# Asd-g/AviSynth-JincResize

Hardware: AMD Instinct MI355X
Metric: Mpix/s per GPU (1080p→4K tap=3 Y8); % HBM-read roofline (higher is better)
Workload: dtype f32

## Files before the change

avisynth-jincresize_amd/csrc/kernel_periodic.hip:

```cpp
#include "device_common.hpp"
#include "knobs.h"
#include <utility>

#pragma clang fp contract(off)

namespace jinc {
namespace {

#include "kernel_periodic_common.inc"

constexpr int kTileCols = 64;

template <int FS, int RG = (FS <= 7 ? 8 : 9)>
struct PeriodicCfg {
    static constexpr int kRowGroups = RG;
    static constexpr int kTileRows = FS * kRowGroups;
    static constexpr int kLdsCols = kTileCols + FS;
    static constexpr int kLdsPitch = kLdsCols + 1;
    static constexpr int kLdsRows = kTileRows + FS;
};

template <typename T, int FS, int RG>
__global__ __launch_bounds__(256) void ewa_periodic_kernel(const PeriodicArgs a, const PlaneIO io) {
    using Cfg = PeriodicCfg<FS, RG>;
// ... 950 lines not shown
            : "v"(w1), "v"(w2), "v"(w3), "s"(c2), "s"(c3), "s"(c4), "s"(c5));
    }
}
#undef JINC_Q7_EVEN
#undef JINC_Q7_ODD

template <int SLOT>
__device__ __forceinline__ void quad2_load_row(f32x2 (&w)[24], const float* p) {
    const f32x2* p2 = reinterpret_cast<const f32x2*>(p);
#pragma unroll
    for (int m = 0; m < 4; ++m) w[4 * SLOT + m] = p2[m];
}

template <int U, uint32_t INNER, int NT>
__device__ __forceinline__ void quad2_pixel6(f32x2 (&acc)[4], const f32x2 (&w)[24], const JINC_CONSTANT f32x2* quad) {
    f32x2 ca[16], cb[16];
    quad_fetch(ca, quad, 0);
#define JINC_QUAD2_STEP(LY, CUR, NEXT)                                                                                        \
    if constexpr (LY < 5) quad_fetch(NEXT, quad, LY + 1);                                                                      \
    __builtin_amdgcn_sched_barrier(0);                                                                                         \
    quad_arrived(CUR);                                                                                                         \
    {                                                                                                                          \
        constexpr int S = 4 * ((U + LY) % 6);                                                                                  \
         \
        if constexpr (NT == 7) {                                             \
                                          \
            quad2_row7_span<(INNER >> (2 * (2 * LY))) & 3u>(acc[0], acc[1], w[S], w[S + 1], w[S + 2], w[S + 3], CUR[0], CUR[1], CUR[2], CUR[3], CUR[4], CUR[5], CUR[6]); \
            quad2_row7_span<(INNER >> (2 * (2 * LY + 1))) & 3u>(acc[2], acc[3], w[S], w[S + 1], w[S + 2], w[S + 3], CUR[8], CUR[9], CUR[10], CUR[11], CUR[12], CUR[13], CUR[14]); \
        } else {                                                                                                               \
        if constexpr ((INNER >> (2 * LY)) & 1u)                                                                                \
            quad2_row6_inner(acc[0], acc[1], w[S], w[S + 1], w[S + 2], CUR[1], CUR[2], CUR[3], CUR[4]);                        \
        else                                                                                                                   \
            quad2_row6(acc[0], acc[1], w[S], w[S + 1], w[S + 2], w[S + 3], CUR[0], CUR[1], CUR[2], CUR[3], CUR[4], CUR[5]);    \
        if constexpr ((INNER >> (2 * LY + 1)) & 1u)                                                                            \
            quad2_row6_inner(acc[2], acc[3], w[S], w[S + 1], w[S + 2], CUR[9], CUR[10], CUR[11], CUR[12]);                     \
        else                                                                                                                   \
            quad2_row6(acc[2], acc[3], w[S], w[S + 1], w[S + 2], w[S + 3], CUR[8], CUR[9], CUR[10], CUR[11], CUR[12], CUR[13]); \
        }                                                                                                                      \
    }                                                                                                                          \
    __builtin_amdgcn_sched_barrier(0);
    JINC_QUAD2_STEP(0, ca, cb)
    JINC_QUAD2_STEP(1, cb, ca)
    JINC_QUAD2_STEP(2, ca, cb)
    JINC_QUAD2_STEP(3, cb, ca)
    JINC_QUAD2_STEP(4, ca, cb)
    JINC_QUAD2_STEP(5, cb, ca)
#undef JINC_QUAD2_STEP
}

template <typename T>
__device__ __forceinline__ void store_quad_buf(BufferRsrc rsrc, uint32_t voffset, uint32_t soffset, f32x2 a, f32x2 b, float peak, bool b_ok) {
    if constexpr (std::is_same_v<T, float>) {
        typedef uint32_t u32x2 __attribute__((ext_vector_type(2)));
        __builtin_amdgcn_raw_buffer_store_b64(__builtin_bit_cast(u32x2, a), rsrc, voffset, soffset, 0);
        if (b_ok) __builtin_amdgcn_raw_buffer_store_b64(__builtin_bit_cast(u32x2, b), rsrc, voffset + 8u, soffset, 0);
    } else if constexpr (std::is_same_v<T, uint8_t>) {
        uint32_t w = __builtin_amdgcn_cvt_pk_u8_f32(a.x, 0u, 0u);
        w = __builtin_amdgcn_cvt_pk_u8_f32(a.y, 1u, w);
        w = __builtin_amdgcn_cvt_pk_u8_f32(b.x, 2u, w);
        w = __builtin_amdgcn_cvt_pk_u8_f32(b.y, 3u, w);
        if (b_ok) __builtin_amdgcn_raw_buffer_store_b32(w, rsrc, voffset, soffset, 0);
        else __builtin_amdgcn_raw_buffer_store_b16(static_cast<uint16_t>(w), rsrc, voffset, soffset, 0);
    } else {
        typedef uint32_t u32x2 __attribute__((ext_vector_type(2)));
        const uint32_t lo = round_pair16<T>(a.x, a.y, peak);
        if (b_ok) {
            const u32x2 v = {lo, round_pair16<T>(b.x, b.y, peak)};
            __builtin_amdgcn_raw_buffer_store_b64(v, rsrc, voffset, soffset, 0);
        } else {
            __builtin_amdgcn_raw_buffer_store_b32(lo, rsrc, voffset, soffset, 0);
        }
    }
}

template <typename T>
__device__ __forceinline__ bool edge_tile_of(const PeriodicArgs& a, int tile_x) {
    if constexpr (is_float_sample_v<T>) return false;
    return a.edge.coeffs != nullptr && ((a.edge.n[0] > 0 && tile_x == a.edge.tile_x[0]) || (a.edge.n[1] > 0 && tile_x == a.edge.tile_x[1]));
}

template <typename T, typename Cfg>
__device__ __forceinline__ void stage_edge_column(const PeriodicArgs& a, const PlaneIO& io, float* tile, int tile_x, const char* sbase, int gx0, int gy0,
                                                  int wave, int lane) {
    static_assert(Cfg::kLdsPitch >= Cfg::kLdsCols + 1 && Cfg::kLdsRows <= 64, "a spare word per tile row, one tile row per lane");
    const bool in_front = (a.edge.n[0] > 0 && tile_x == a.edge.tile_x[0] && a.edge.lds_col[0] < 0) || (a.edge.n[1] > 0 && tile_x == a.edge.tile_x[1] && a.edge.lds_col[1] < 0);
    if (in_front && wave == 0 && lane < Cfg::kLdsRows && gx0 > 0) {
        int gy = gy0 + lane;
        gy = gy < a.src_h ? gy : a.src_h - 1;
        tile[lane * Cfg::kLdsPitch - 1] = to_float(reinterpret_cast<const T*>(sbase + static_cast<size_t>(gy) * io.src_pitch)[gx0 - 1]);
    }
}

template <typename T, typename Cfg, int NR, int NC, int ES = 1>
__device__ __forceinline__ void quad2_edge_columns(const PeriodicArgs& a, const PlaneIO& io, const float* tile, int tile_x, int j0, int wave, int lane,
                                                   BufferRsrc drsrc) {
    constexpr int NCP = (NC + 3) & ~3;
    for (int s = 0; s < 2; ++s) {
        const int n = a.edge.n[s];
        if (n <= 0 || tile_x != a.edge.tile_x[s]) continue;
        const int q = wave & 1, half = (n + 1) >> 1;
        const int k_begin = (wave >> 1) * half, k_end = k_begin + half < n ? k_begin + half : n;
        if (k_begin >= k_end) continue;
        const bool live = lane < Cfg::kTileRows && j0 + lane < a.nj;
        static_assert(Cfg::kLdsRows <= 64, "one tile row per lane");
        const float* wp = tile + ((lane < Cfg::kLdsRows ? lane : 0) * Cfg::kLdsPitch + a.edge.lds_col[s]) * ES;
        float w[NR][NC];
#pragma unroll
        for (int lx = 0; lx < NC; ++lx) w[0][lx] = wp[lx * ES];
#pragma unroll
        for (int ly = 1; ly < NR; ++ly)
#pragma unroll
            for (int lx = 0; lx < NC; ++lx)
                w[ly][lx] = __builtin_bit_cast(float, __builtin_amdgcn_update_dpp(0, __builtin_bit_cast(int, w[ly - 1][lx]), 0x130, 0xf, 0xf, false));
        const uint32_t row_off = static_cast<uint32_t>(a.iy0 + 2 * (j0 + lane) + q) * static_cast<uint32_t>(io.dst_pitch);
        for (int k0 = k_begin; k0 < k_end; k0 += 4) {
            const int nk = k_end - k0 < 4 ? k_end - k0 : 4;
            float r[4];
#pragma unroll
            for (int k = 0; k < 4; ++k) {
                r[k] = 0.f;
                if (k < nk) {
                    const JINC_CONSTANT float* cs = (const JINC_CONSTANT float*)(a.edge.coeffs) + ((s * PeriodicArgs::EdgeColumns::kMaxPerSide + k0 + k) * 2 + q) * (NR * NCP);
                    float acc = 0.f;
#pragma unroll
                    for (int ly = 0; ly < NR; ++ly)
#pragma unroll
                        for (int lx = 0; lx < NC; ++lx) acc = acc + w[ly][lx] * cs[ly * NCP + lx];
                    r[k] = acc;
                }
            }
            if (!live) continue;
            const uint32_t voff = row_off + static_cast<uint32_t>(a.edge.x0[s] + k0) * static_cast<uint32_t>(sizeof(T));
            if (nk == 4) {
                if constexpr (std::is_same_v<T, uint8_t>) {
                    uint32_t v = __builtin_amdgcn_cvt_pk_u8_f32(r[0], 0u, 0u);
                    v = __builtin_amdgcn_cvt_pk_u8_f32(r[1], 1u, v);
                    v = __builtin_amdgcn_cvt_pk_u8_f32(r[2], 2u, v);
                    v = __builtin_amdgcn_cvt_pk_u8_f32(r[3], 3u, v);
                    __builtin_amdgcn_raw_buffer_store_b32(v, drsrc, voff, 0, 0);
                } else {
                    typedef uint32_t u32x2 __attribute__((ext_vector_type(2)));
                    const u32x2 v = {round_pair_u16(r[0], r[1], io.peak), round_pair_u16(r[2], r[3], io.peak)};
                    __builtin_amdgcn_raw_buffer_store_b64(v, drsrc, voff, 0, 0);
                }
            } else {
#pragma unroll
                for (int k = 0; k < 3; ++k)
                    if (k < nk) store_sample_buf<T>(drsrc, voff + static_cast<uint32_t>(k * sizeof(T)), 0, r[k], io.peak);
            }
        }
    }
}

struct Quad2ShareCfg {
    static constexpr int kTileCols = 128;
    static constexpr int kBlocksPerWave = 2;
    static constexpr int kTileRows = 4 * 2 * kBlocksPerWave;
    static constexpr int kLdsCols = kTileCols + 6;
    static constexpr int kLdsPitch = 136;
    static constexpr int kLdsRows = kTileRows + 5;
    static constexpr int kLdsFloats = 2 * (2 + kLdsRows * kLdsPitch);
};

template <int RG>
__host__ __device__ inline bool quad2_share_runs(const PlaneIO& io) { return RG == 8 || io.nframes > 1; }

constexpr uint32_t quad2_share_outs(int r, int c, int k) {
    uint32_t m = 0;
    for (int oy = 0; oy < 4; ++oy)
        for (int ox = 0; ox < 4; ++ox) {
            const int ly = r - (oy >> 1), lx = c - (ox >> 1);
            if (ly < 0 || ly > 5 || lx < 0 || lx > 5) continue;
            if (quad2_share_class(quad2_share_m(ox & 1, lx), quad2_share_m(oy & 1, ly)) == k) m |= 1u << (4 * oy + ox);
        }
    return m;
}

template <int R, int C, int K>
__device__ __forceinline__ void quad2_share_mul(f32x2& t, f32x2 s, const f32x2 (&w)[kQuad2ShareClasses / 2]) {
    if constexpr (quad2_share_outs(R, C, K) != 0) {
        if constexpr (K & 1)
            asm("v_pk_mul_f32 %0, %1, %2 op_sel:[0,1] op_sel_hi:[1,1]" : "=v"(t) : "v"(s), "s"(w[K >> 1]));
        else
            asm("v_pk_mul_f32 %0, %1, %2 op_sel_hi:[1,0]" : "=v"(t) : "v"(s), "s"(w[K >> 1]));
    }
}
template <int R, int C, int K>
__device__ __forceinline__ void quad2_share_adds(f32x2 (&acc)[16], f32x2 t) {
    constexpr uint32_t outs = quad2_share_outs(R, C, K);
#pragma unroll
    for (int o = 0; o < 16; ++o)
        if constexpr (outs != 0)
            if ((outs >> o) & 1u) asm("v_pk_add_f32 %0, %0, %1" : "+v"(acc[o]) : "v"(t));
}
template <int R, int C, int... K>
__device__ __forceinline__ void quad2_share_sample(f32x2 (&acc)[16], f32x2 s, const f32x2 (&w)[kQuad2ShareClasses / 2], std::integer_sequence<int, K...>) {
    f32x2 t[kQuad2ShareClasses];
    (quad2_share_mul<R, C, K>(t[K], s, w), ...);
    (quad2_share_adds<R, C, K>(acc, t[K]), ...);
}
template <int R, int... C>
__device__ __forceinline__ void quad2_share_row(f32x2 (&acc)[16], const f32x2 (&row)[8], const f32x2 (&w)[kQuad2ShareClasses / 2], std::integer_sequence<int, C...>) {
    (quad2_share_sample<R, C>(acc, row[C], w, std::make_integer_sequence<int, kQuad2ShareClasses>{}), ...);
}

template <typename T>
__device__ __forceinline__ void quad2_share_body(const PeriodicArgs& a, const PlaneIO& io, float* lds) {
    using Cfg = Quad2ShareCfg;
    typedef float f32x4 __attribute__((ext_vector_type(4)));
    f32x2* const tile = reinterpret_cast<f32x2*>(lds) + 2;
    const int lane = threadIdx.x & 63;
    const int wave = __builtin_amdgcn_readfirstlane(threadIdx.x >> 6);
    int tile_x, tile_y;
    swizzled_tile(tile_x, tile_y);
    const int i0 = tile_x * Cfg::kTileCols;
    const int j0 = tile_y * Cfg::kTileRows;
    const size_t f0 = 2 * static_cast<size_t>(blockIdx.z);
    const bool f1_ok = f0 + 1 < static_cast<size_t>(io.nframes);
    const size_t f1 = f1_ok ? f0 + 1 : f0;
    const bool edge_tile = edge_tile_of<T>(a, tile_x);
    {
        const int gx0 = a.min_sx + i0;
        const int gy0 = a.min_sy + j0;
        const char* sb0 = static_cast<const char*>(io.src) + f0 * io.src_frame_stride;
        const char* sb1 = static_cast<const char*>(io.src) + f1 * io.src_frame_stride;
        constexpr int kRowsPerWave = (Cfg::kLdsRows + 3) / 4;
        constexpr int kColsPerLane = (Cfg::kLdsCols + 63) / 64;
        T s0[kRowsPerWave][kColsPerLane], s1[kRowsPerWave][kColsPerLane];
#pragma unroll
        for (int i = 0; i < kRowsPerWave; ++i) {
            int gy = gy0 + wave + 4 * i;
            gy = gy < a.src_h ? gy : a.src_h - 1;
            const T* r0 = reinterpret_cast<const T*>(sb0 + static_cast<size_t>(gy) * io.src_pitch);
            const T* r1 = reinterpret_cast<const T*>(sb1 + static_cast<size_t>(gy) * io.src_pitch);
#pragma unroll
            for (int k = 0; k < kColsPerLane; ++k) {
                int gx = gx0 + lane + 64 * k;
                gx = gx < a.src_w ? gx : a.src_w - 1;
                s0[i][k] = r0[gx];
                s1[i][k] = r1[gx];
            }
        }
#pragma unroll
        for (int i = 0; i < kRowsPerWave; ++i) {
            const int r = wave + 4 * i;
#pragma unroll
            for (int k = 0; k < kColsPerLane; ++k) {
                const int c = lane + 64 * k;
                if (r < Cfg::kLdsRows && c < Cfg::kLdsCols) tile[r * Cfg::kLdsPitch + c] = f32x2{to_float(s0[i][k]), to_float(s1[i][k])};
            }
        }
        const bool in_front = edge_tile && ((a.edge.n[0] > 0 && tile_x == a.edge.tile_x[0] && a.edge.lds_col[0] < 0) ||
                                            (a.edge.n[1] > 0 && tile_x == a.edge.tile_x[1] && a.edge.lds_col[1] < 0));
        if (in_front && wave == 0 && lane < Cfg::kLdsRows && gx0 > 0) {
            int gy = gy0 + lane;
            gy = gy < a.src_h ? gy : a.src_h - 1;
            tile[lane * Cfg::kLdsPitch - 1] = f32x2{to_float(reinterpret_cast<const T*>(sb0 + static_cast<size_t>(gy) * io.src_pitch)[gx0 - 1]),
                                                    to_float(reinterpret_cast<const T*>(sb1 + static_cast<size_t>(gy) * io.src_pitch)[gx0 - 1])};
        }
    }
    __syncthreads();
    const uint32_t plane_bytes = static_cast<uint32_t>(io.dst_pitch) * a.dst_h;
    const BufferRsrc d0 = make_rsrc(static_cast<char*>(io.dst) + f0 * io.dst_frame_stride, plane_bytes);
    const BufferRsrc d1 = make_rsrc(static_cast<char*>(io.dst) + f1 * io.dst_frame_stride, plane_bytes);
    if (edge_tile) {
        quad2_edge_columns<T, Cfg, 6, 7, 2>(a, io, reinterpret_cast<const float*>(tile), tile_x, j0, wave, lane, d0);
        if (f1_ok) quad2_edge_columns<T, Cfg, 6, 7, 2>(a, io, reinterpret_cast<const float*>(tile) + 1, tile_x, j0, wave, lane, d1);
    }
    const int ia = i0 + 2 * lane;
    if (ia >= a.ni) return;
    const bool b_ok = ia + 1 < a.ni;
    f32x2 w[kQuad2ShareClasses / 2];
#pragma unroll
    for (int k = 0; k < kQuad2ShareClasses / 2; ++k) w[k] = f32x2{a.share_w[2 * k], a.share_w[2 * k + 1]};
    const uint32_t xoff = static_cast<uint32_t>(a.ix0 + 2 * ia) * static_cast<uint32_t>(sizeof(T));
    for (int blk = 0; blk < Cfg::kBlocksPerWave; ++blk) {
        const int jb = 2 * (wave * Cfg::kBlocksPerWave + blk);
        if (j0 + jb >= a.nj) break;
        const f32x2* wb = tile + jb * Cfg::kLdsPitch + 2 * lane;
        f32x2 acc[16];
#pragma unroll
        for (int o = 0; o < 16; ++o) acc[o] = f32x2{0.f, 0.f};
#define JINC_SHARE_ROW(R)                                                                                 \
    {                                                                                                     \
        const f32x4* p4 = reinterpret_cast<const f32x4*>(wb + (R) * Cfg::kLdsPitch);                      \
        f32x2 row[8];                                                                                     \
        _Pragma("unroll") for (int m = 0; m < 4; ++m) {                                                   \
            const f32x4 v = p4[m];                                                                        \
            row[2 * m] = f32x2{v.x, v.y};                                                                 \
            row[2 * m + 1] = f32x2{v.z, v.w};                                                             \
        }                                                                                                 \
        quad2_share_row<R>(acc, row, w, std::make_integer_sequence<int, 7>{});                            \
    }
        JINC_SHARE_ROW(0) JINC_SHARE_ROW(1) JINC_SHARE_ROW(2) JINC_SHARE_ROW(3) JINC_SHARE_ROW(4) JINC_SHARE_ROW(5) JINC_SHARE_ROW(6)
#undef JINC_SHARE_ROW
#pragma unroll
        for (int pr = 0; pr < 2; ++pr) {
            const int j = j0 + jb + pr;
            if (j >= a.nj) break;
#pragma unroll
            for (int q = 0; q < 2; ++q) {
                const uint32_t so = static_cast<uint32_t>(a.iy0 + 2 * j + q) * static_cast<uint32_t>(io.dst_pitch);
                const f32x2* r = acc + 4 * (2 * pr + q);
                store_quad_buf<T>(d0, xoff, so, f32x2{r[0].x, r[1].x}, f32x2{r[2].x, r[3].x}, io.peak, b_ok);
                if (f1_ok) store_quad_buf<T>(d1, xoff, so, f32x2{r[0].y, r[1].y}, f32x2{r[2].y, r[3].y}, io.peak, b_ok);
            }
        }
    }
}

constexpr uint32_t kQuad2InnerTap3 = PeriodicArgs::kQuadInnerTap3;
template <typename T, int RG, uint32_t INNER, int NT = 6>
__global__ __launch_bounds__(256, 6) void ewa_periodic_quad2_kernel(const PeriodicArgs a, const PlaneIO io) {
    using Cfg = Quad2Cfg<RG>;
    constexpr int FS = Cfg::FS;
    static_assert(RG % 4 == 0, "the four waves of a workgroup take RG / 4 row groups each");
    constexpr bool kShare = !is_float_sample_v<T> && INNER == kQuad2InnerTap3 && NT == 6;
    constexpr int kWords = 2 + Cfg::kLdsRows * Cfg::kLdsPitch;
    if constexpr (kShare && RG == 8) {
        __shared__ __attribute__((aligned(16))) float share_words[Quad2ShareCfg::kLdsFloats];
        quad2_share_body<T>(a, io, share_words);
        return;
    }
    __shared__ __attribute__((aligned(16))) float tile_words[kShare && Quad2ShareCfg::kLdsFloats > kWords ? Quad2ShareCfg::kLdsFloats : kWords];
    if constexpr (kShare) {
        if (quad2_share_runs<RG>(io)) {
            quad2_share_body<T>(a, io, tile_words);
            return;
        }
    }
    float* const tile = tile_words + 2;

    const int lane = threadIdx.x & 63;
    const int wave = __builtin_amdgcn_readfirstlane(threadIdx.x >> 6);
    int tile_x, tile_y;
    swizzled_tile(tile_x, tile_y);
    const int i0 = tile_x * Cfg::kTileCols;
    const int j0 = tile_y * Cfg::kTileRows;
    const size_t frame = blockIdx.z;
    if (skips_frame(a, frame)) return;
    const bool edge_tile = edge_tile_of<T>(a, tile_x);
    {
        const int gx0 = a.min_sx + i0;
        const int gy0 = a.min_sy + j0;
        const char* sbase = static_cast<const char*>(io.src) + frame * io.src_frame_stride;
        constexpr int kRowsPerWave = (Cfg::kLdsRows + 3) / 4;
        constexpr int kColsPerLane = (Cfg::kLdsCols + 63) / 64;
        T staged[kRowsPerWave][kColsPerLane];
        NonFinite<T> nonfinite(a, frame);
#pragma unroll
        for (int i = 0; i < kRowsPerWave; ++i) {
            int gy = gy0 + wave + 4 * i;
            gy = gy < a.src_h ? gy : a.src_h - 1;
            const T* srow = reinterpret_cast<const T*>(sbase + static_cast<size_t>(gy) * io.src_pitch);
#pragma unroll
            for (int k = 0; k < kColsPerLane; ++k) {
                int gx = gx0 + lane + 64 * k;
                gx = gx < a.src_w ? gx : a.src_w - 1;
                staged[i][k] = srow[gx];
            }
        }
#pragma unroll
        for (int i = 0; i < kRowsPerWave; ++i) {
            const int r = wave + 4 * i;
#pragma unroll
            for (int k = 0; k < kColsPerLane; ++k) {
                const int c = lane + 64 * k;
                if (r < Cfg::kLdsRows && c < Cfg::kLdsCols) tile[r * Cfg::kLdsPitch + c] = nonfinite.take(staged[i][k]);
            }
        }
        if constexpr (!is_float_sample_v<T>) {
            if (edge_tile) stage_edge_column<T, Cfg>(a, io, tile, tile_x, sbase, gx0, gy0, wave, lane);
        }
    }
    __syncthreads();
    const BufferRsrc drsrc = make_rsrc(static_cast<char*>(io.dst) + frame * io.dst_frame_stride,
                                       static_cast<uint32_t>(io.dst_pitch) * a.dst_h);
    if constexpr (!is_float_sample_v<T>) {
        if (edge_tile) quad2_edge_columns<T, Cfg, 6, 7>(a, io, tile, tile_x, j0, wave, lane, drsrc);
    }
    const int ia = i0 + 2 * lane;
    if (ia >= a.ni) return;
    const bool b_ok = ia + 1 < a.ni;

    const JINC_CONSTANT f32x2* quad = (const JINC_CONSTANT f32x2*)(a.quad);
    const float* base = tile + 2 * lane;
    const uint32_t xoff = static_cast<uint32_t>(a.ix0 + 2 * ia) * static_cast<uint32_t>(sizeof(T));

    constexpr int kGroupsPerWave = RG / 4;
    const int g_first = wave * kGroupsPerWave;
    if (j0 + g_first * FS >= a.nj) return;
    f32x2 win[24];
    {
        const float* wb = base + (g_first * FS) * Cfg::kLdsPitch;
        quad2_load_row<0>(win, wb + 0 * Cfg::kLdsPitch);
        quad2_load_row<1>(win, wb + 1 * Cfg::kLdsPitch);
        quad2_load_row<2>(win, wb + 2 * Cfg::kLdsPitch);
        quad2_load_row<3>(win, wb + 3 * Cfg::kLdsPitch);
        quad2_load_row<4>(win, wb + 4 * Cfg::kLdsPitch);
    }
    for (int g = g_first; g < g_first + kGroupsPerWave; ++g) {
        if (j0 + g * FS >= a.nj) break;
        const float* gbase = base + (g * FS) * Cfg::kLdsPitch;
#define JINC_QUAD2_ROW(U)                                                                                          \
    {                                                                                                              \
        quad2_load_row<(U + FS - 1) % FS>(win, gbase + (U + FS - 1) * Cfg::kLdsPitch);                              \
        f32x2 acc[4] = {{0.f, 0.f}, {0.f, 0.f}, {0.f, 0.f}, {0.f, 0.f}};                                            \
        uint32_t zero;                                                                                              \
        asm volatile("s_mov_b32 %0, 0" : "=s"(zero));  \
        quad2_pixel6<U, INNER, NT>(acc, win, quad + zero);                                                          \
        const int j = j0 + g * FS + U;                                                                              \
        if (j < a.nj) {                                                                                             \
            const uint32_t so = static_cast<uint32_t>(a.iy0 + 2 * j) * io.dst_pitch;                                \
            store_quad_buf<T>(drsrc, xoff, so, acc[0], acc[1], io.peak, b_ok);                                      \
            store_quad_buf<T>(drsrc, xoff, so + static_cast<uint32_t>(io.dst_pitch), acc[2], acc[3], io.peak, b_ok); \
        }                                                                                                           \
    }
        JINC_QUAD2_ROW(0) JINC_QUAD2_ROW(1) JINC_QUAD2_ROW(2) JINC_QUAD2_ROW(3) JINC_QUAD2_ROW(4) JINC_QUAD2_ROW(5)
#undef JINC_QUAD2_ROW
    }
}

template <int RG>
struct Quad2x8Cfg {
    static constexpr int FS = 8;
    static constexpr int kTileCols = 128;
    static constexpr int kTileRows = FS * RG;
    static constexpr int kLdsCols = kTileCols + FS;
    static constexpr int kLdsPitch = 138;
    static constexpr int kLdsRows = kTileRows + FS - 1;
};

__device__ __forceinline__ void quad2_row8(f32x2& acc_a, f32x2& acc_b, f32x2 w0, f32x2 w1, f32x2 w2, f32x2 w3, f32x2 w4, f32x2 c0, f32x2 c1,
                                           f32x2 c2, f32x2 c3, f32x2 c4, f32x2 c5, f32x2 c6, f32x2 c7) {
    f32x2 ta, tb;
#define JINC_LO(T, W, C) "v_pk_mul_f32 " T ", " W ", " C " op_sel_hi:[0,1]\n\t"
#define JINC_HI(T, W, C) "v_pk_mul_f32 " T ", " W ", " C " op_sel:[1,0] op_sel_hi:[1,1]\n\t"
#define JINC_ADD2 "v_pk_add_f32 %0, %0, %2\n\tv_pk_add_f32 %1, %1, %3\n\t"
    asm(JINC_LO("%2", "%4", "%9") JINC_HI("%3", "%4", "%9") JINC_ADD2
        JINC_HI("%2", "%4", "%10") JINC_LO("%3", "%5", "%10") JINC_ADD2
        JINC_LO("%2", "%5", "%11") JINC_HI("%3", "%5", "%11") JINC_ADD2
        JINC_HI("%2", "%5", "%12") JINC_LO("%3", "%6", "%12") JINC_ADD2
        JINC_LO("%2", "%6", "%13") JINC_HI("%3", "%6", "%13") JINC_ADD2
        JINC_HI("%2", "%6", "%14") JINC_LO("%3", "%7", "%14") JINC_ADD2
        JINC_LO("%2", "%7", "%15") JINC_HI("%3", "%7", "%15") JINC_ADD2
        JINC_HI("%2", "%7", "%16") JINC_LO("%3", "%8", "%16")
        "v_pk_add_f32 %0, %0, %2\n\tv_pk_add_f32 %1, %1, %3"
        : "+v"(acc_a), "+v"(acc_b), "=&v"(ta), "=&v"(tb)
        : "v"(w0), "v"(w1), "v"(w2), "v"(w3), "v"(w4), "s"(c0), "s"(c1), "s"(c2), "s"(c3), "s"(c4), "s"(c5), "s"(c6), "s"(c7));
#undef JINC_LO
#undef JINC_HI
#undef JINC_ADD2
}

template <int SLOT>
__device__ __forceinline__ void quad2x8_load_row(f32x2 (&w)[40], const float* p) {
    const f32x2* p2 = reinterpret_cast<const f32x2*>(p);
#pragma unroll
    for (int m = 0; m < 5; ++m) w[5 * SLOT + m] = p2[m];
}

template <int U, uint32_t TR8>
__device__ __forceinline__ void quad2_pixel8(f32x2 (&acc)[4], const f32x2 (&w)[40], const JINC_CONSTANT f32x2* quad) {
    f32x2 ca[16], cb[16];
    quad_fetch(ca, quad, 0);
#define JINC_QUAD2X8_STEP(LY, CUR, NEXT)                                                                                                  \
    if constexpr (LY < 7) quad_fetch(NEXT, quad, LY + 1);                                                                                  \
    __builtin_amdgcn_sched_barrier(0);                                                                                                     \
    quad_arrived(CUR);                                                                                                                     \
    {                                                                                                                                      \
        constexpr int S = 5 * ((U + LY) % 8);                                                                                              \
        if constexpr (quad8_trim_of(TR8, LY, 0) == 2)                                                                                      \
            quad2_row8_t2(acc[0], acc[1], w[S + 1], w[S + 2], w[S + 3], CUR[2], CUR[3], CUR[4], CUR[5]);                                   \
        else if constexpr (quad8_trim_of(TR8, LY, 0) == 1)                                                                                 \
            quad2_row8_t1(acc[0], acc[1], w[S], w[S + 1], w[S + 2], w[S + 3], CUR[1], CUR[2], CUR[3], CUR[4], CUR[5], CUR[6]);             \
        else                                                                                                                               \
            quad2_row8(acc[0], acc[1], w[S], w[S + 1], w[S + 2], w[S + 3], w[S + 4], CUR[0], CUR[1], CUR[2], CUR[3], CUR[4], CUR[5],       \
                       CUR[6], CUR[7]);                                                                                                    \
        if constexpr (quad8_trim_of(TR8, LY, 1) == 2)                                                                                      \
            quad2_row8_t2(acc[2], acc[3], w[S + 1], w[S + 2], w[S + 3], CUR[10], CUR[11], CUR[12], CUR[13]);                               \
// ... 302 lines not shown
    if (skips_frame(a, frame)) return;

    {
        const int gx0 = a.min_sx + i0;
        const int gy0 = a.min_sy + j0;
        const char* sbase = static_cast<const char*>(io.src) + frame * io.src_frame_stride;
        constexpr int kRowsPerWave = (Cfg::kRows + Cfg::kWaves - 1) / Cfg::kWaves;
        constexpr int kColsPerLane = (Cfg::kCols + 63) / 64;
        T staged[kRowsPerWave][kColsPerLane];
        NonFinite<T> nonfinite(a, frame);
#pragma unroll
        for (int i = 0; i < kRowsPerWave; ++i) {
            int gy = gy0 + wave + Cfg::kWaves * i;
            gy = gy < a.src_h ? gy : a.src_h - 1;
            const T* srow = reinterpret_cast<const T*>(sbase + static_cast<size_t>(gy) * io.src_pitch);
#pragma unroll
            for (int k = 0; k < kColsPerLane; ++k) {
                int gx = gx0 + lane + 64 * k;
                gx = gx < a.src_w ? gx : a.src_w - 1;
                staged[i][k] = srow[gx];
            }
        }
#pragma unroll
        for (int i = 0; i < kRowsPerWave; ++i) {
            const int r = wave + Cfg::kWaves * i;
#pragma unroll
            for (int k = 0; k < kColsPerLane; ++k) {
                const int c = lane + 64 * k;
                if (r < Cfg::kRows && c < Cfg::kCols)
                    tile[(c % K) * Cfg::kPlaneStride + r * Cfg::kPlane + c / K] = nonfinite.take(staged[i][k]);
            }
        }
    }
    __syncthreads();

    const BufferRsrc dframe = make_rsrc(static_cast<char*>(io.dst) + frame * io.dst_frame_stride,
                                        static_cast<uint32_t>(io.dst_pitch) * a.dst_h);
    const int nphase = a.px * a.py;
    const int nitems = nphase * Cfg::kChunks;
    const int cols_valid = a.ni - (i0 + K * lane);
    if (cols_valid <= 0) return;
    for (int item = wave; item < nitems; item += Cfg::kWaves) {
        const int ch = item / nphase;
        const int ph = item - ch * nphase;
        const int q = ph / a.px;
        const int p = ph - q * a.px;
        const int j = j0 + ch * R;
        const int rows_valid = a.nj - j;
        if (rows_valid <= 0) continue;
        const int nrows = a.rows_ny ? a.rows_ny : FS;
        const JINC_CONSTANT float* cs =
            (const JINC_CONSTANT float*)(a.coeffs + static_cast<size_t>(a.set[ph]) * (static_cast<size_t>(nrows) * padded_row(FS)));
        const unsigned base = ((a.start_y[q] - a.min_sy) + ch * R) * Cfg::kPlane + lane;
        const int y0 = a.iy0 + a.py * j + q;
        const unsigned x0 = a.ix0 + a.px * (i0 + K * lane) + p;
        const JINC_CONSTANT int32_t* row_trim = a.row_trim ? (const JINC_CONSTANT int32_t*)(a.row_trim) + ph * 32 : nullptr;
        if (a.start_x[p] - a.min_sx)
            rows_item<T, FS, KC, 1>(tile, base, cs, row_trim, nrows, dframe, io.dst_pitch, io.peak, y0, a.py, rows_valid, x0, a.px, cols_valid);
        else
            rows_item<T, FS, KC, 0>(tile, base, cs, row_trim, nrows, dframe, io.dst_pitch, io.peak, y0, a.py, rows_valid, x0, a.px, cols_valid);
    }
}

template <typename T, int FS, int RG = PeriodicCfg<FS>::kRowGroups>
int launch_periodic_t(const PeriodicArgs& pa, const PlaneIO& io, hipStream_t stream) {
    using Cfg = PeriodicCfg<FS, RG>;
    dim3 grid((pa.ni + kTileCols - 1) / kTileCols, (pa.nj + Cfg::kTileRows - 1) / Cfg::kTileRows, io.nframes);
    hipLaunchKernelGGL((ewa_periodic_kernel<T, FS, RG>), grid, dim3(256, 1, 1), 0, stream, pa, io);
    knobs::note_instance("ewa_periodic_kernel", "%s, %d, %d", knobs::type_name<T>(), FS, RG);
    return static_cast<int>(hipGetLastError());
}

template <typename T, int FS, int RG>
int launch_periodic_pk_t(const PeriodicArgs& pa, const PlaneIO& io, hipStream_t stream) {
    using Cfg = PeriodicPkCfg<FS, RG>;
    dim3 grid((pa.ni + Cfg::kTileCols - 1) / Cfg::kTileCols, (pa.nj + Cfg::kTileRows - 1) / Cfg::kTileRows, io.nframes);
    hipLaunchKernelGGL((ewa_periodic_pk_kernel<T, FS, RG>), grid, dim3(256, 1, 1), 0, stream, pa, io);
    knobs::note_instance("ewa_periodic_pk_kernel", "%s, %d, %d", knobs::type_name<T>(), FS, RG);
    return static_cast<int>(hipGetLastError());
}

template <typename T, int RG>
int launch_periodic_quad_t(const PeriodicArgs& pa, const PlaneIO& io, hipStream_t stream) {
    using Cfg = PeriodicCfg<7, RG>;
    dim3 grid((pa.ni + kTileCols - 1) / kTileCols, (pa.nj + Cfg::kTileRows - 1) / Cfg::kTileRows, io.nframes);
    hipLaunchKernelGGL((ewa_periodic_quad_kernel<T, RG>), grid, dim3(256, 1, 1), 0, stream, pa, io);
    knobs::note_instance("ewa_periodic_quad_kernel", "%s, %d", knobs::type_name<T>(), RG);
    return static_cast<int>(hipGetLastError());
}

template <typename T, int RG>
int launch_periodic_quad9_t(const PeriodicArgs& pa, const PlaneIO& io, hipStream_t stream) {
    using Cfg = PeriodicCfg<9, RG>;
    dim3 grid((pa.ni + kTileCols - 1) / kTileCols, (pa.nj + Cfg::kTileRows - 1) / Cfg::kTileRows, io.nframes);
    hipLaunchKernelGGL((ewa_periodic_quad9_kernel<T, RG>), grid, dim3(256, 1, 1), 0, stream, pa, io);
    knobs::note_instance("ewa_periodic_quad9_kernel", "%s, %d", knobs::type_name<T>(), RG);
    return static_cast<int>(hipGetLastError());
}

template <typename T, int RG>
int launch_periodic_quad8_t(const PeriodicArgs& pa, const PlaneIO& io, hipStream_t stream) {
    using Cfg = PeriodicCfg<8, RG>;
    dim3 grid((pa.ni + kTileCols - 1) / kTileCols, (pa.nj + Cfg::kTileRows - 1) / Cfg::kTileRows, io.nframes);
    const bool pattern = quad8_pattern_fits(pa.quad_trim8, kQuad8TrimTap4);
    if (pattern)
        hipLaunchKernelGGL((ewa_periodic_quad8_kernel<T, RG, kQuad8TrimTap4>), grid, dim3(256, 1, 1), 0, stream, pa, io);
    else
        hipLaunchKernelGGL((ewa_periodic_quad8_kernel<T, RG, 0u>), grid, dim3(256, 1, 1), 0, stream, pa, io);
    knobs::note_instance("ewa_periodic_quad8_kernel", "%s, %d, %uu", knobs::type_name<T>(), RG, pattern ? kQuad8TrimTap4 : 0u);
    return static_cast<int>(hipGetLastError());
}

template <typename T, int RG>
int launch_periodic_quad2x8_t(const PeriodicArgs& pa, const PlaneIO& io, hipStream_t stream) {
    using Cfg = Quad2x8Cfg<RG>;
    dim3 grid((pa.ni + Cfg::kTileCols - 1) / Cfg::kTileCols, (pa.nj + Cfg::kTileRows - 1) / Cfg::kTileRows, io.nframes);
    if (pa.quad_taps == 9) {
        const uint64_t span = quad_span9_fits(pa.quad_span7, kQuadSpan9Mpeg2) ? kQuadSpan9Mpeg2 : quad_span9_fits(pa.quad_span7, kQuadSpan9Mpeg2Swapped) ? kQuadSpan9Mpeg2Swapped : 0;
        if (span == kQuadSpan9Mpeg2)
            hipLaunchKernelGGL((ewa_periodic_quad2x8_kernel<T, RG, 0u, 9, kQuadSpan9Mpeg2>), grid, dim3(256, 1, 1), 0, stream, pa, io);
        else if (span == kQuadSpan9Mpeg2Swapped)
            hipLaunchKernelGGL((ewa_periodic_quad2x8_kernel<T, RG, 0u, 9, kQuadSpan9Mpeg2Swapped>), grid, dim3(256, 1, 1), 0, stream, pa, io);
        else
            hipLaunchKernelGGL((ewa_periodic_quad2x8_kernel<T, RG, 0u, 9, 0>), grid, dim3(256, 1, 1), 0, stream, pa, io);
        knobs::note_instance("ewa_periodic_quad2x8_kernel", "%s, %d, 0u, 9, %lluul", knobs::type_name<T>(), RG, static_cast<unsigned long long>(span));
        return static_cast<int>(hipGetLastError());
    }
    const bool pattern = quad8_pattern_fits(pa.quad_trim8, kQuad8TrimTap4);
    if (pattern)
        hipLaunchKernelGGL((ewa_periodic_quad2x8_kernel<T, RG, kQuad8TrimTap4>), grid, dim3(256, 1, 1), 0, stream, pa, io);
    else
        hipLaunchKernelGGL((ewa_periodic_quad2x8_kernel<T, RG, 0u>), grid, dim3(256, 1, 1), 0, stream, pa, io);
    knobs::note_instance("ewa_periodic_quad2x8_kernel", "%s, %d, %uu, 8, 0ul", knobs::type_name<T>(), RG, pattern ? kQuad8TrimTap4 : 0u);
    return static_cast<int>(hipGetLastError());
}

template <typename T, int RG>
int launch_periodic_quad2_t(const PeriodicArgs& pa, const PlaneIO& io, hipStream_t stream) {
    using Cfg = Quad2Cfg<RG>;
    dim3 grid((pa.ni + Cfg::kTileCols - 1) / Cfg::kTileCols, (pa.nj + Cfg::kTileRows - 1) / Cfg::kTileRows, io.nframes);
    if (pa.quad_taps == 7 && quad_span7_fits(pa.quad_span7, PeriodicArgs::kQuadSpan7Mpeg2)) {
        hipLaunchKernelGGL((ewa_periodic_quad2_kernel<T, RG, PeriodicArgs::kQuadSpan7Mpeg2, 7>), grid, dim3(256, 1, 1), 0, stream, pa, io);
        knobs::note_instance("ewa_periodic_quad2_kernel", "%s, %d, %uu, 7", knobs::type_name<T>(), RG, PeriodicArgs::kQuadSpan7Mpeg2);
    } else if (pa.quad_taps == 7 && quad_span7_fits(pa.quad_span7, PeriodicArgs::kQuadSpan7Mpeg2Swapped)) {
        hipLaunchKernelGGL((ewa_periodic_quad2_kernel<T, RG, PeriodicArgs::kQuadSpan7Mpeg2Swapped, 7>), grid, dim3(256, 1, 1), 0, stream, pa, io);
        knobs::note_instance("ewa_periodic_quad2_kernel", "%s, %d, %uu, 7", knobs::type_name<T>(), RG, PeriodicArgs::kQuadSpan7Mpeg2Swapped);
    } else if (pa.quad_taps == 7) {
        hipLaunchKernelGGL((ewa_periodic_quad2_kernel<T, RG, 0u, 7>), grid, dim3(256, 1, 1), 0, stream, pa, io);
        knobs::note_instance("ewa_periodic_quad2_kernel", "%s, %d, 0u, 7", knobs::type_name<T>(), RG);
    } else if ((pa.quad_inner & kQuad2InnerTap3) == kQuad2InnerTap3) {
        bool share = false;
        if constexpr (!is_float_sample_v<T>) share = true;
        if (share && pa.quad_share) {
            if (quad2_share_runs<RG>(io))
                grid = dim3((pa.ni + Quad2ShareCfg::kTileCols - 1) / Quad2ShareCfg::kTileCols, (pa.nj + Quad2ShareCfg::kTileRows - 1) / Quad2ShareCfg::kTileRows,
                            (io.nframes + 1) / 2);
        } else if (share) {
            hipLaunchKernelGGL((ewa_periodic_quad2_kernel<T, RG, 0u>), grid, dim3(256, 1, 1), 0, stream, pa, io);
            knobs::note_instance("ewa_periodic_quad2_kernel", "%s, %d, 0u, 6", knobs::type_name<T>(), RG);
            return static_cast<int>(hipGetLastError());
        }
        hipLaunchKernelGGL((ewa_periodic_quad2_kernel<T, RG, kQuad2InnerTap3>), grid, dim3(256, 1, 1), 0, stream, pa, io);
        knobs::note_instance("ewa_periodic_quad2_kernel", "%s, %d, %uu, 6", knobs::type_name<T>(), RG, kQuad2InnerTap3);
    } else {
        hipLaunchKernelGGL((ewa_periodic_quad2_kernel<T, RG, 0u>), grid, dim3(256, 1, 1), 0, stream, pa, io);
        knobs::note_instance("ewa_periodic_quad2_kernel", "%s, %d, 0u, 6", knobs::type_name<T>(), RG);
    }
    return static_cast<int>(hipGetLastError());
}

template <typename T, int FS, int KC>
int launch_rows_k(const PeriodicArgs& pa, const PlaneIO& io, hipStream_t stream) {
    using Cfg = RowsCfg<FS, KC>;
    dim3 grid((pa.ni + Cfg::kTileCols - 1) / Cfg::kTileCols, (pa.nj + Cfg::kTileRows - 1) / Cfg::kTileRows, io.nframes);
    hipLaunchKernelGGL((ewa_periodic_rows_kernel<T, FS, KC>), grid, dim3(Cfg::kThreads, 1, 1), 0, stream, pa, io);
    knobs::note_instance("ewa_periodic_rows_kernel", "%s, %d, %d", knobs::type_name<T>(), FS, KC);
    return static_cast<int>(hipGetLastError());
}

template <typename T, int FS>
int launch_rows_t(const PeriodicArgs& pa, const PlaneIO& io, hipStream_t stream) {
    const long long cover4 = (pa.ni + 255) / 256 * 256LL, cover3 = (pa.ni + 191) / 192 * 192LL;
    if (cover3 * 100 < cover4 * 97) return launch_rows_k<T, FS, 3>(pa, io, stream);
    return launch_rows_k<T, FS, 4>(pa, io, stream);
}

template <typename T>
int launch_periodic_fs(const PeriodicArgs& pa, int fs, const PlaneIO& io, hipStream_t stream, int variant) {
    if ((variant == 5 || variant == 6) && fs == 6 && pa.quad)
        return variant == 5 ? launch_periodic_quad2_t<T, 8>(pa, io, stream) : launch_periodic_quad2_t<T, 4>(pa, io, stream);
    if (variant == 7 && fs == 8 && pa.quad) return launch_periodic_quad2x8_t<T, 4>(pa, io, stream);
    if (pa.edge.coeffs) return static_cast<int>(hipErrorInvalidValue);
    if ((variant == 5 || variant == 6) && fs == 8 && pa.quad)
        return variant == 5 ? launch_periodic_quad8_t<T, 8>(pa, io, stream) : launch_periodic_quad8_t<T, 4>(pa, io, stream);
    if ((variant == 5 || variant == 6) && fs == 7 && pa.quad)
        return variant == 5 ? launch_periodic_quad_t<T, 8>(pa, io, stream) : launch_periodic_quad_t<T, 4>(pa, io, stream);
    if ((variant == 5 || variant == 6) && fs == 9 && pa.quad)
        return launch_periodic_quad9_t<T, 4>(pa, io, stream);
    if (variant == 3 && fs == 7) return launch_periodic_pk_t<T, 7, 4>(pa, io, stream);
    if (variant == 4 && fs == 7) return launch_periodic_pk_t<T, 7, 8>(pa, io, stream);
    if (variant == 2 && fs == 7) return launch_periodic_t<T, 7, 4>(pa, io, stream);
    if (variant == 2 && fs == 9) return launch_periodic_t<T, 9, 6>(pa, io, stream);
    if (variant == 2 && fs == 6) return launch_periodic_t<T, 6, 4>(pa, io, stream);
    if (variant == 2 && fs == 8) return launch_periodic_t<T, 8, 5>(pa, io, stream);
    if (variant == 1) {
        if (fs == 7) return launch_rows_t<T, 7>(pa, io, stream);
        if (fs == 9) return launch_rows_t<T, 9>(pa, io, stream);
        if (fs == 6) return launch_rows_t<T, 6>(pa, io, stream);
        if (fs == 8) return launch_rows_t<T, 8>(pa, io, stream);
    }
    switch (fs) {
        case 3: return launch_rows_t<T, 3>(pa, io, stream);
        case 4: return launch_rows_t<T, 4>(pa, io, stream);
        case 5: return launch_rows_t<T, 5>(pa, io, stream);
        case 6: return launch_periodic_t<T, 6>(pa, io, stream);
        case 7: return launch_periodic_t<T, 7>(pa, io, stream);
        case 8: return launch_periodic_t<T, 8>(pa, io, stream);
        case 9: return launch_periodic_t<T, 9>(pa, io, stream);
        case 10: return launch_rows_t<T, 10>(pa, io, stream);
        case 11: return launch_rows_t<T, 11>(pa, io, stream);
        case 12: return launch_rows_t<T, 12>(pa, io, stream);
        case 13: return launch_rows_t<T, 13>(pa, io, stream);
        case 14: return launch_rows_t<T, 14>(pa, io, stream);
        case 15: return launch_rows_t<T, 15>(pa, io, stream);
        case 16: return launch_rows_t<T, 16>(pa, io, stream);
        case 17: return launch_rows_t<T, 17>(pa, io, stream);
        default: return static_cast<int>(hipErrorInvalidValue);
    }
}


}

bool periodic_supported(int fs, int px, int py, int sx, int sy) {
    if (sx != 1 || sy != 1) return false;
    if (px < 1 || py < 1 || px > 8 || py > 8) return false;
    return fs >= 3 && fs <= 17 && (fs & 1);
}

int launch_periodic(const PeriodicArgs& args, int fs, const PlaneIO& io, void* stream, int variant) {
    if (args.ni <= 0 || args.nj <= 0 || io.nframes <= 0) return 0;
    if (args.rowpair && knobs::flag(JINC_KNOB_ROWS_PAIR, true)) {
        const int taps = args.quad_taps ? args.quad_taps : fs;
        const bool auto_variant = variant == 0 || variant == 2 || variant == 5 || variant == 6 || variant == 7;
        if (args.rowpair_n == taps && !args.edge.coeffs &&
            ((fs >= 10 && variant == 0) || (fs < 10 && auto_variant && knobs::geti(JINC_KNOB_ROWPAIR_SMALL, 0) == 1)))
            return launch_rowpair(args, io, stream);
    }
    hipStream_t s = static_cast<hipStream_t>(stream);
    switch (io.sample_bytes) {
        case 1: return launch_periodic_fs<uint8_t>(args, fs, io, s, variant);
        case 2:
            if (io.sample_kind == kSampleHalf) return launch_periodic_fs<half_t>(args, fs, io, s, variant);
            return launch_periodic_fs<uint16_t>(args, fs, io, s, variant);
        default: return launch_periodic_fs<float>(args, fs, io, s, variant);
    }
}


}
```

Baseline: 1.049 million.

## Use taller register strips in the shared-weight quad2 path for RG=8

For RG=8, the shared-weight quad2 path now has each wave compute one 8-row strip instead of two 2-row blocks. This means the 5-row filter halo is re-read from LDS and re-multiplied once per 8 output rows rather than once per 2. Each output row is stored as soon as its last input row has been accumulated. The multiply and add phases are interleaved with a configurable lead so that the packed multiplies run ahead of the adds. The larger accumulator array (64 f32x2) raises register pressure, so the launch-bounds occupancy hint for this instance drops from 6 to 4 blocks, and the tile becomes 32 rows tall.

```diff
diff --git a/avisynth-jincresize_amd/csrc/kernel_periodic.hip b/avisynth-jincresize_amd/csrc/kernel_periodic.hip
--- a/avisynth-jincresize_amd/csrc/kernel_periodic.hip
+++ b/avisynth-jincresize_amd/csrc/kernel_periodic.hip
@@ -1126,62 +1126,93 @@
     }
 }
 
-struct Quad2ShareCfg {
+template <int H, int StripsPerWave, int MulLead>
+struct Quad2ShareTile {
     static constexpr int kTileCols = 128;
-    static constexpr int kBlocksPerWave = 2;
-    static constexpr int kTileRows = 4 * 2 * kBlocksPerWave;
+    static constexpr int kStripRows = H;
+    static constexpr int kStripsPerWave = StripsPerWave;
+    static constexpr int kMulLead = MulLead;
+    static constexpr int kTileRows = 4 * H * StripsPerWave;
     static constexpr int kLdsCols = kTileCols + 6;
     static constexpr int kLdsPitch = 136;
     static constexpr int kLdsRows = kTileRows + 5;
     static constexpr int kLdsFloats = 2 * (2 + kLdsRows * kLdsPitch);
+    static_assert(8 * H <= 64, "a strip's outputs index one 64-bit mask");
 };
+template <int RG>
+using Quad2ShareCfg = std::conditional_t<RG == 8, Quad2ShareTile<8, 1, 1>, Quad2ShareTile<2, 2, kQuad2ShareClasses>>;
 
 template <int RG>
 __host__ __device__ inline bool quad2_share_runs(const PlaneIO& io) { return RG == 8 || io.nframes > 1; }
 
-constexpr uint32_t quad2_share_outs(int r, int c, int k) {
-    uint32_t m = 0;
-    for (int oy = 0; oy < 4; ++oy)
+template <int H>
+constexpr uint64_t quad2_share_outs(int r, int c, int k) {
+    uint64_t m = 0;
+    for (int oy = 0; oy < 2 * H; ++oy)
         for (int ox = 0; ox < 4; ++ox) {
             const int ly = r - (oy >> 1), lx = c - (ox >> 1);
             if (ly < 0 || ly > 5 || lx < 0 || lx > 5) continue;
-            if (quad2_share_class(quad2_share_m(ox & 1, lx), quad2_share_m(oy & 1, ly)) == k) m |= 1u << (4 * oy + ox);
+            if (quad2_share_class(quad2_share_m(ox & 1, lx), quad2_share_m(oy & 1, ly)) == k) m |= uint64_t{1} << (4 * oy + ox);
         }
     return m;
 }
 
-template <int R, int C, int K>
+template <int H, int R, int C, int K>
 __device__ __forceinline__ void quad2_share_mul(f32x2& t, f32x2 s, const f32x2 (&w)[kQuad2ShareClasses / 2]) {
-    if constexpr (quad2_share_outs(R, C, K) != 0) {
+    if constexpr (quad2_share_outs<H>(R, C, K) != 0) {
         if constexpr (K & 1)
             asm("v_pk_mul_f32 %0, %1, %2 op_sel:[0,1] op_sel_hi:[1,1]" : "=v"(t) : "v"(s), "s"(w[K >> 1]));
         else
             asm("v_pk_mul_f32 %0, %1, %2 op_sel_hi:[1,0]" : "=v"(t) : "v"(s), "s"(w[K >> 1]));
     }
 }
-template <int R, int C, int K>
-__device__ __forceinline__ void quad2_share_adds(f32x2 (&acc)[16], f32x2 t) {
-    constexpr uint32_t outs = quad2_share_outs(R, C, K);
-#pragma unroll
-    for (int o = 0; o < 16; ++o)
+template <int H, int R, int C, int K>
+__device__ __forceinline__ void quad2_share_adds(f32x2 (&acc)[8 * H], f32x2 t) {
+    constexpr uint64_t outs = quad2_share_outs<H>(R, C, K);
+#pragma unroll
+    for (int o = 0; o < 8 * H; ++o)
         if constexpr (outs != 0)
             if ((outs >> o) & 1u) asm("v_pk_add_f32 %0, %0, %1" : "+v"(acc[o]) : "v"(t));
 }
-template <int R, int C, int... K>
-__device__ __forceinline__ void quad2_share_sample(f32x2 (&acc)[16], f32x2 s, const f32x2 (&w)[kQuad2ShareClasses / 2], std::integer_sequence<int, K...>) {
+template <typename Cfg, int R, int C, int K>
+__device__ __forceinline__ void quad2_share_step(f32x2 (&acc)[8 * Cfg::kStripRows], f32x2 (&t)[kQuad2ShareClasses], f32x2 s,
+                                                 const f32x2 (&w)[kQuad2ShareClasses / 2]) {
+    if constexpr (K < kQuad2ShareClasses) quad2_share_mul<Cfg::kStripRows, R, C, K>(t[K], s, w);
+    if constexpr (K >= Cfg::kMulLead) quad2_share_adds<Cfg::kStripRows, R, C, K - Cfg::kMulLead>(acc, t[K - Cfg::kMulLead]);
+}
+template <typename Cfg, int R, int C, int... K>
+__device__ __forceinline__ void quad2_share_sample(f32x2 (&acc)[8 * Cfg::kStripRows], f32x2 s, const f32x2 (&w)[kQuad2ShareClasses / 2],
+                                                   std::integer_sequence<int, K...>) {
     f32x2 t[kQuad2ShareClasses];
-    (quad2_share_mul<R, C, K>(t[K], s, w), ...);
-    (quad2_share_adds<R, C, K>(acc, t[K]), ...);
-}
-template <int R, int... C>
-__device__ __forceinline__ void quad2_share_row(f32x2 (&acc)[16], const f32x2 (&row)[8], const f32x2 (&w)[kQuad2ShareClasses / 2], std::integer_sequence<int, C...>) {
-    (quad2_share_sample<R, C>(acc, row[C], w, std::make_integer_sequence<int, kQuad2ShareClasses>{}), ...);
-}
-
-template <typename T>
+    (quad2_share_step<Cfg, R, C, K>(acc, t, s, w), ...);
+}
+template <typename Cfg, int R, int... C>
+__device__ __forceinline__ void quad2_share_row(f32x2 (&acc)[8 * Cfg::kStripRows], const f32x2* wb, const f32x2 (&w)[kQuad2ShareClasses / 2],
+                                                std::integer_sequence<int, C...>) {
+    typedef float f32x4 __attribute__((ext_vector_type(4)));
+    if constexpr (R < Cfg::kStripRows) {
+#pragma unroll
+        for (int o = 0; o < 8; ++o) acc[8 * R + o] = f32x2{0.f, 0.f};
+    }
+    const f32x4* p4 = reinterpret_cast<const f32x4*>(wb + R * Cfg::kLdsPitch);
+    f32x2 row[8];
+#pragma unroll
+    for (int m = 0; m < 4; ++m) {
+        const f32x4 v = p4[m];
+        row[2 * m] = f32x2{v.x, v.y};
+        row[2 * m + 1] = f32x2{v.z, v.w};
+    }
+    (quad2_share_sample<Cfg, R, C>(acc, row[C], w, std::make_integer_sequence<int, kQuad2ShareClasses + Cfg::kMulLead>{}), ...);
+}
+template <typename Cfg, int... R, typename Store>
+__device__ __forceinline__ void quad2_share_strip(f32x2 (&acc)[8 * Cfg::kStripRows], const f32x2* wb, const f32x2 (&w)[kQuad2ShareClasses / 2],
+                                                  std::integer_sequence<int, R...>, Store&& store) {
+    ((quad2_share_row<Cfg, R>(acc, wb, w, std::make_integer_sequence<int, 7>{}), store(std::integral_constant<int, R - 5>{})), ...);
+}
+
+template <typename T, int RG>
 __device__ __forceinline__ void quad2_share_body(const PeriodicArgs& a, const PlaneIO& io, float* lds) {
-    using Cfg = Quad2ShareCfg;
-    typedef float f32x4 __attribute__((ext_vector_type(4)));
+    using Cfg = Quad2ShareCfg<RG>;
     f32x2* const tile = reinterpret_cast<f32x2*>(lds) + 2;
     const int lane = threadIdx.x & 63;
     const int wave = __builtin_amdgcn_readfirstlane(threadIdx.x >> 6);
@@ -1248,58 +1279,50 @@
 #pragma unroll
     for (int k = 0; k < kQuad2ShareClasses / 2; ++k) w[k] = f32x2{a.share_w[2 * k], a.share_w[2 * k + 1]};
     const uint32_t xoff = static_cast<uint32_t>(a.ix0 + 2 * ia) * static_cast<uint32_t>(sizeof(T));
-    for (int blk = 0; blk < Cfg::kBlocksPerWave; ++blk) {
-        const int jb = 2 * (wave * Cfg::kBlocksPerWave + blk);
+    for (int st = 0; st < Cfg::kStripsPerWave; ++st) {
+        const int jb = Cfg::kStripRows * (wave * Cfg::kStripsPerWave + st);
         if (j0 + jb >= a.nj) break;
         const f32x2* wb = tile + jb * Cfg::kLdsPitch + 2 * lane;
-        f32x2 acc[16];
-#pragma unroll
-        for (int o = 0; o < 16; ++o) acc[o] = f32x2{0.f, 0.f};
-#define JINC_SHARE_ROW(R)                                                                                 \
-    {                                                                                                     \
-        const f32x4* p4 = reinterpret_cast<const f32x4*>(wb + (R) * Cfg::kLdsPitch);                      \
-        f32x2 row[8];                                                                                     \
-        _Pragma("unroll") for (int m = 0; m < 4; ++m) {                                                   \
-            const f32x4 v = p4[m];                                                                        \
-            row[2 * m] = f32x2{v.x, v.y};                                                                 \
-            row[2 * m + 1] = f32x2{v.z, v.w};                                                             \
-        }                                                                                                 \
-        quad2_share_row<R>(acc, row, w, std::make_integer_sequence<int, 7>{});                            \
-    }
-        JINC_SHARE_ROW(0) JINC_SHARE_ROW(1) JINC_SHARE_ROW(2) JINC_SHARE_ROW(3) JINC_SHARE_ROW(4) JINC_SHARE_ROW(5) JINC_SHARE_ROW(6)
-#undef JINC_SHARE_ROW
-#pragma unroll
-        for (int pr = 0; pr < 2; ++pr) {
-            const int j = j0 + jb + pr;
-            if (j >= a.nj) break;
-#pragma unroll
-            for (int q = 0; q < 2; ++q) {
-                const uint32_t so = static_cast<uint32_t>(a.iy0 + 2 * j + q) * static_cast<uint32_t>(io.dst_pitch);
-                const f32x2* r = acc + 4 * (2 * pr + q);
-                store_quad_buf<T>(d0, xoff, so, f32x2{r[0].x, r[1].x}, f32x2{r[2].x, r[3].x}, io.peak, b_ok);
-                if (f1_ok) store_quad_buf<T>(d1, xoff, so, f32x2{r[0].y, r[1].y}, f32x2{r[2].y, r[3].y}, io.peak, b_ok);
-            }
-        }
+        f32x2 acc[8 * Cfg::kStripRows];
+        quad2_share_strip<Cfg>(acc, wb, w, std::make_integer_sequence<int, Cfg::kStripRows + 5>{}, [&](auto PR) {
+            constexpr int pr = decltype(PR)::value;
+            if constexpr (pr >= 0) {
+                const int j = j0 + jb + pr;
+                if (j < a.nj) {
+#pragma unroll
+                    for (int q = 0; q < 2; ++q) {
+                        const uint32_t so = static_cast<uint32_t>(a.iy0 + 2 * j + q) * static_cast<uint32_t>(io.dst_pitch);
+                        const f32x2* r = acc + 4 * (2 * pr + q);
+                        store_quad_buf<T>(d0, xoff, so, f32x2{r[0].x, r[1].x}, f32x2{r[2].x, r[3].x}, io.peak, b_ok);
+                        if (f1_ok) store_quad_buf<T>(d1, xoff, so, f32x2{r[0].y, r[1].y}, f32x2{r[2].y, r[3].y}, io.peak, b_ok);
+                    }
+                }
+            }
+        });
     }
 }
 
 constexpr uint32_t kQuad2InnerTap3 = PeriodicArgs::kQuadInnerTap3;
+template <typename T, uint32_t INNER, int NT>
+constexpr bool quad2_share_instance() { return !is_float_sample_v<T> && INNER == kQuad2InnerTap3 && NT == 6; }
 template <typename T, int RG, uint32_t INNER, int NT = 6>
-__global__ __launch_bounds__(256, 6) void ewa_periodic_quad2_kernel(const PeriodicArgs a, const PlaneIO io) {
+__global__ __launch_bounds__(256, (quad2_share_instance<T, INNER, NT>() && RG == 8 ? 4 : 6)) void ewa_periodic_quad2_kernel(const PeriodicArgs a,
+                                                                                                                       const PlaneIO io) {
     using Cfg = Quad2Cfg<RG>;
     constexpr int FS = Cfg::FS;
     static_assert(RG % 4 == 0, "the four waves of a workgroup take RG / 4 row groups each");
-    constexpr bool kShare = !is_float_sample_v<T> && INNER == kQuad2InnerTap3 && NT == 6;
+    constexpr bool kShare = quad2_share_instance<T, INNER, NT>();
+    using ShareCfg = Quad2ShareCfg<RG>;
     constexpr int kWords = 2 + Cfg::kLdsRows * Cfg::kLdsPitch;
     if constexpr (kShare && RG == 8) {
-        __shared__ __attribute__((aligned(16))) float share_words[Quad2ShareCfg::kLdsFloats];
-        quad2_share_body<T>(a, io, share_words);
+        __shared__ __attribute__((aligned(16))) float share_words[ShareCfg::kLdsFloats];
+        quad2_share_body<T, RG>(a, io, share_words);
         return;
     }
-    __shared__ __attribute__((aligned(16))) float tile_words[kShare && Quad2ShareCfg::kLdsFloats > kWords ? Quad2ShareCfg::kLdsFloats : kWords];
+    __shared__ __attribute__((aligned(16))) float tile_words[kShare && ShareCfg::kLdsFloats > kWords ? ShareCfg::kLdsFloats : kWords];
     if constexpr (kShare) {
         if (quad2_share_runs<RG>(io)) {
-            quad2_share_body<T>(a, io, tile_words);
+            quad2_share_body<T, RG>(a, io, tile_words);
             return;
         }
     }
@@ -1908,8 +1931,9 @@
         bool share = false;
         if constexpr (!is_float_sample_v<T>) share = true;
         if (share && pa.quad_share) {
+            using ShareCfg = Quad2ShareCfg<RG>;
             if (quad2_share_runs<RG>(io))
-                grid = dim3((pa.ni + Quad2ShareCfg::kTileCols - 1) / Quad2ShareCfg::kTileCols, (pa.nj + Quad2ShareCfg::kTileRows - 1) / Quad2ShareCfg::kTileRows,
+                grid = dim3((pa.ni + ShareCfg::kTileCols - 1) / ShareCfg::kTileCols, (pa.nj + ShareCfg::kTileRows - 1) / ShareCfg::kTileRows,
                             (io.nframes + 1) / 2);
         } else if (share) {
             hipLaunchKernelGGL((ewa_periodic_quad2_kernel<T, RG, 0u>), grid, dim3(256, 1, 1), 0, stream, pa, io);
```

Measured after the change: 1.187 million (median of 6 runs). 13.1% higher.
